# facebookresearch/FRL-Distributed-ML-Scaffold

Measured on NVIDIA H100. Metric: samples/sec (whole box) on synthetic 2-task Problem, higher is better.
Workload: dtype bf16

## Files before the change

frl-distributed-ml-scaffold_b200/_native.py:

```python
import ctypes as C
import os
import subprocess
from typing import Optional, Sequence

import torch

_HERE = os.path.dirname(os.path.abspath(__file__))
CSRC_DIR = os.path.join(_HERE, "csrc")
LIB_PATH = os.path.join(CSRC_DIR, "libfrl_b200.so")

F32, BF16, U8, I64 = 0, 1, 2, 3
LOSS_MSE, LOSS_CE = 0, 1
FP8_E4M3, FP8_E5M2 = 0, 1
FP8_DTYPE = {FP8_E4M3: torch.float8_e4m3fn, FP8_E5M2: torch.float8_e5m2}
MAX_TASKS = 8

_DTYPE_CODE = {torch.float32: F32, torch.bfloat16: BF16, torch.uint8: U8, torch.bool: U8,
               torch.int64: I64}


class NativeLibraryError(RuntimeError):
    pass


class TaskDesc(C.Structure):
    _fields_ = [
        ("kind", C.c_int32), ("out_dtype", C.c_int32), ("tgt_dtype", C.c_int32),
        ("ignore_index", C.c_int32),
        ("out", C.c_void_p), ("tgt", C.c_void_p), ("mask", C.c_void_p), ("dout", C.c_void_p),
        ("rows", C.c_int64), ("cols", C.c_int64), ("mask_inner", C.c_int64),
        ("weight", C.c_float), ("_pad", C.c_float),
    ]


class GradSeg(C.Structure):
    _fields_ = [("g", C.c_void_p), ("arena_off", C.c_int64), ("numel", C.c_int64),
                ("g_dtype", C.c_int32), ("_pad", C.c_int32)]


_vp, _i, _i64, _f, _d = C.c_void_p, C.c_int, C.c_int64, C.c_float, C.c_double
SIGNATURES = {
    "frl_abi_version": (_i, []),
    "frl_last_error": (C.c_char_p, []),
    "frl_launch_count": (C.c_uint64, []),
    "frl_launch_count_reset": (None, []),
    "frl_device_sm_count": (_i, []),
    "frl_device_arch": (_i, []),
# ... 29 lines not shown
    "frl_gather_lines": (_i, [_vp, _i64, _i64, _vp, _i64, _vp, _vp, _i64, _i64, _i, _i, _vp]),
    "frl_gather_pool_create": (_vp, [_i]),
    "frl_gather_pool_destroy": (None, [_vp]),
    "frl_gather_pool_threads": (_i, [_vp]),
    "frl_gather_pool_submit": (_i64, [_vp, _vp, _i64, _vp, _vp, _i64, _i64]),
    "frl_gather_pool_submit_f32_to_bf16": (_i64, [_vp, _vp, _i64, _vp, _vp, _i64, _i64]),
    "frl_gather_pool_wait": (_i, [_vp, _i64]),
    "frl_nvls_sgd": (_i, [_vp, _vp, _vp, _vp, _i64, _i, _i, _vp, _i, _vp, _i, _d, _d, _d, _d, _d, _vp, _i, _i, _i, _vp]),
    "frl_nvls_adam": (_i, [_vp, _vp, _vp, _vp, _vp, _vp, _i64, _i, _i, _vp, _i, _vp, _i, _d, _d, _d, _d, _d,
                           _i64, _d, _vp, _i, _i, _vp]),
    "frl_nvls_rmsprop": (_i, [_vp, _vp, _vp, _vp, _vp, _i64, _i, _i, _vp, _i, _vp, _i, _d, _d, _d, _d, _d, _d,
                              _vp, _i, _i, _vp]),
    "frl_nvls_barrier": (_i, [_vp, _i, _i, _i, _vp]),
    "frl_fp8_amax": (_i, [_vp, _i64, _i, _vp, _vp]),
    "frl_fp8_quantize": (_i, [_vp, _i64, _i64, _i, _vp, _i, _vp, _vp, _vp, _vp]),
}

_lib: Optional[C.CDLL] = None


def build(verbose: bool = False) -> str:
    cmd = ["make", "-C", CSRC_DIR, "-j8"]
    res = subprocess.run(cmd, capture_output=True, text=True)
    if verbose or res.returncode != 0:
        print(res.stdout)
        print(res.stderr)
    if res.returncode != 0:
        raise NativeLibraryError("building libfrl_b200.so failed:\n" + res.stderr[-4000:])
    return LIB_PATH

# ... 301 lines not shown
    _check(lib().frl_fp8_amax(_ptr(src), src.numel(), dtype_code(src.dtype), _ptr(amax_out), _stream()),
           "frl_fp8_amax")


def fp8_quantize(src, amax, fmt: int, dst=None, dst_t=None, inv_scale_out=None) -> None:
    rows, cols = src.shape
    want = FP8_DTYPE[fmt]
    assert src.is_contiguous() and amax.dtype == torch.float32 and inv_scale_out.dtype == torch.float32
    assert dst is None or (dst.shape == (rows, cols) and dst.dtype == want and dst.is_contiguous())
    assert dst_t is None or (dst_t.shape == (cols, rows) and dst_t.dtype == want and dst_t.is_contiguous())
    _check(lib().frl_fp8_quantize(_ptr(src), rows, cols, dtype_code(src.dtype), _ptr(amax), fmt, _ptr(dst),
                                  _ptr(dst_t), _ptr(inv_scale_out), _stream()), "frl_fp8_quantize")



def gather_rows(src_pinned, idx_dev, dst, max_blocks: int = 64) -> None:
    assert src_pinned.is_pinned() and src_pinned.is_contiguous() and dst.is_contiguous()
    row_bytes = src_pinned[0].numel() * src_pinned.element_size() if src_pinned.shape[0] else 0
    _check(lib().frl_gather_rows(_ptr(src_pinned), src_pinned.shape[0], _ptr(idx_dev), _ptr(dst),
                                 idx_dev.numel(), row_bytes, max_blocks, _stream()),
           "frl_gather_rows")


def _row_bytes(src) -> int:
    return src[0].numel() * src.element_size() if src.shape[0] else 0


def gather_rows_tma(src_pinned, idx_dev, dst, max_blocks: int = 0) -> None:
    assert src_pinned.is_pinned() and src_pinned.is_contiguous() and dst.is_contiguous()
    _check(lib().frl_gather_rows_tma(_ptr(src_pinned), src_pinned.shape[0], _ptr(idx_dev), _ptr(dst),
# ... 77 lines not shown
```

frl-distributed-ml-scaffold_b200/arena_linear.py:

```python
import os
import types
from collections import Counter
from typing import List, Optional

import torch
import torch.nn as nn
import torch.nn.functional as F

from . import _native
from .types import Precision

KERNELS = _native

FP8_MULTIPLE = 16


def fp8_site_qualifies(uses_lp: bool, in_features: int, out_features: int) -> bool:
    return bool(uses_lp) and in_features % FP8_MULTIPLE == 0 and out_features % FP8_MULTIPLE == 0


def fp8_call_qualifies(x: torch.Tensor) -> bool:
    if x.dim() == 0 or x.shape[-1] == 0 or x.dtype not in (torch.bfloat16, torch.float32):
        return False
    m = x.numel() // x.shape[-1]
    return m > 0 and m % FP8_MULTIPLE == 0 and (not x.is_contiguous() or x.data_ptr() % 16 == 0)


# ... 33 lines not shown
            KERNELS.colsum(dz2, pipe.arena.grad_view(site.bslot),
                           accumulate=not site.bstate.first_touch(pipe.step_id))
        site.backward_done(pipe)
        return dx, None, None, None, None
    dw = _fp8_mm(dztq, xtq, sdz, sx) if ctx.needs_input_grad[1] else None
    db = dz2.sum(0) if (ctx.has_bias and ctx.needs_input_grad[2]) else None
    return dx, dw, db, None, None


class _ArenaLinearFn(torch.autograd.Function):
    @staticmethod
    def forward(ctx, x, weight, bias, site):
        ctx.site = site
        ctx.has_bias = bias is not None
        ctx.save_for_backward(x, weight)
        if x.dim() <= 2:
            return F.linear(x, weight, bias)
        y = torch.empty(*x.shape[:-1], weight.shape[0], dtype=x.dtype, device=x.device)
        x2 = x.reshape(-1, x.shape[-1])
        if bias is not None:
            torch.addmm(bias, x2, weight.t(), out=y.view(-1, weight.shape[0]))
        else:
            torch.mm(x2, weight.t(), out=y.view(-1, weight.shape[0]))
        return y

    @staticmethod
    @torch.autograd.function.once_differentiable
    def backward(ctx, dy):
        x, weight = ctx.saved_tensors
        site = ctx.site
        dx = dy.matmul(weight) if ctx.needs_input_grad[0] else None
        dy2 = dy.reshape(-1, dy.shape[-1])
        x2 = x.reshape(-1, x.shape[-1])
        pipe = site.pipeline
        if pipe is not None and pipe.step_open:
            site.weight_grad(pipe, dy2, x2)
            if ctx.has_bias and site.bslot is not None:
                if not dy2.is_contiguous():
                    dy2 = dy2.contiguous()
                KERNELS.colsum(dy2, pipe.arena.grad_view(site.bslot),
                               accumulate=not site.bstate.first_touch(pipe.step_id))
            site.backward_done(pipe)
            return dx, None, None, None
        dw = dy2.t().mm(x2) if ctx.needs_input_grad[1] else None
        db = dy2.sum(0) if (ctx.has_bias and ctx.needs_input_grad[2]) else None
        return dx, dw, db, None


class _ArenaLinearReluFn(torch.autograd.Function):

    @staticmethod
    def forward(ctx, x, weight, bias, site):
        ctx.site = site
        x2 = x.reshape(-1, x.shape[-1])
        y = torch.empty(*x.shape[:-1], weight.shape[0], dtype=x.dtype, device=x.device)
        torch._addmm_activation(bias, x2, weight.t(), use_gelu=False, out=y.view(-1, weight.shape[0]))
        ctx.save_for_backward(x, weight, y)
        return y

    @staticmethod
    @torch.autograd.function.once_differentiable
    def backward(ctx, dy):
        x, weight, y = ctx.saved_tensors
        site = ctx.site
        dy2 = dy.reshape(-1, dy.shape[-1])
        if not dy2.is_contiguous():
            dy2 = dy2.contiguous()
        y2 = y.reshape(-1, y.shape[-1])
        x2 = x.reshape(-1, x.shape[-1])
        pipe = site.pipeline
        if pipe is not None and pipe.step_open and (dy2.is_cuda or KERNELS is not _native):
            dz = torch.empty_like(dy2)
            KERNELS.drelu_colsum(dy2, y2, dz, pipe.arena.grad_view(site.bslot),
                                 accumulate=not site.bstate.first_touch(pipe.step_id))
            dx = dz.matmul(weight).view_as(x) if ctx.needs_input_grad[0] else None
            site.weight_grad(pipe, dz, x2)
            site.backward_done(pipe)
            return dx, None, None, None
        dz = dy2 * (y2 > 0).to(dy2.dtype)
        dx = dz.matmul(weight).view_as(x) if ctx.needs_input_grad[0] else None
        dw = dz.t().mm(x2) if ctx.needs_input_grad[1] else None
        db = dz.sum(0) if ctx.needs_input_grad[2] else None
        return dx, dw, db, None


class _Fp8LinearFn(torch.autograd.Function):

    @staticmethod
    def forward(ctx, x, weight, bias, site, for_backward):
        ctx.site = site
        ctx.has_bias = bias is not None
        ctx.x_shape = x.shape
        xq, xtq, sx, wq, wtq, sw = _fp8_operands(x, weight, for_backward)
        y = torch.empty(*x.shape[:-1], weight.shape[0], dtype=torch.bfloat16, device=x.device)
        _fp8_mm(xq, wq, sx, sw, bias=bias, out=y.view(-1, weight.shape[0]))
        if for_backward:
# ... 37 lines not shown
        if pipe is not None and pipe.step_open:
            dz = torch.empty_like(dy2)
            KERNELS.drelu_colsum(dy2, y2, dz, pipe.arena.grad_view(site.bslot),
                                 accumulate=not site.bstate.first_touch(pipe.step_id))
            return _fp8_backward(ctx, site, dz, False)
        return _fp8_backward(ctx, site, dy2 * (y2 > 0).to(dy2.dtype), True)


class _ArenaMultiHeadFn(torch.autograd.Function):

    @staticmethod
    def forward(ctx, x, site, *params):
        ctx.site = site
        ctx.save_for_backward(x)
        ctx.n_heads = len(params) // 2
        return tuple(F.linear(x, params[2 * i], params[2 * i + 1]) for i in range(ctx.n_heads))

    @staticmethod
    @torch.autograd.function.once_differentiable
    def backward(ctx, *dys):
        (x,) = ctx.saved_tensors
        site = ctx.site
        pipe = site.pipeline
        dy = torch.cat(dys, dim=1)
        dx = dy.matmul(site.weight_cat()) if ctx.needs_input_grad[0] else None
        none = (None,) * (2 * ctx.n_heads)
        if pipe is not None and pipe.step_open:
            gw = site.grad_weight_cat()
            if site.heads[0].wstate.first_touch(pipe.step_id):
                torch.mm(dy.t(), x, out=gw)
            else:
                gw.addmm_(dy.t(), x)
            for h in site.heads[1:]:
                h.wstate.first_touch(pipe.step_id)
            gb = site.grad_bias_cat()
            if gb is not None:
                first = site.heads[0].bstate.first_touch(pipe.step_id)
                for h in site.heads[1:]:
                    h.bstate.first_touch(pipe.step_id)
                KERNELS.colsum(dy, gb, accumulate=not first)
            else:
                for h, dyi in zip(site.heads, dys):
                    KERNELS.colsum(dyi.contiguous(), pipe.arena.grad_view(h.bslot),
                                   accumulate=not h.bstate.first_touch(pipe.step_id))
            for h in site.heads:
                h.backward_done(pipe)
            return (dx, None) + none
        grads = []
        for i, dyi in enumerate(dys):
            grads += [dyi.t().mm(x) if ctx.needs_input_grad[2 + 2 * i] else None,
                      dyi.sum(0) if ctx.needs_input_grad[3 + 2 * i] else None]
        return (dx, None) + tuple(grads)


class MultiHeadSite:

    def __init__(self, model, heads: List["LinearSite"], pipeline) -> None:
        self.model = model
        self.heads = heads
        self.pipeline = pipeline
        arena = pipeline.arena
        self.rows = sum(h.module.out_features for h in heads)
        self.cols = heads[0].module.in_features
        self._w_lo = heads[0].wslot.offset
        ends = [h.wslot.end for h in heads]
        starts = [h.wslot.offset for h in heads]
        assert all(e == s for e, s in zip(ends[:-1], starts[1:])), "head weights are not adjacent"
        self._w_hi = ends[-1]
        b_adjacent = all(h.bslot.end == n.bslot.offset for h, n in zip(heads[:-1], heads[1:]))
        self._b = (heads[0].bslot.offset, heads[-1].bslot.end) if b_adjacent else None
        self._arena = arena

    def weight_cat(self) -> torch.Tensor:
        a = self._arena
        store = a.lp if self.heads[0].wslot.uses_lp else a.master
        return store[self._w_lo:self._w_hi].view(self.rows, self.cols)

    def grad_weight_cat(self) -> torch.Tensor:
        return self._arena.grad[self._w_lo:self._w_hi].view(self.rows, self.cols)

    def grad_bias_cat(self) -> Optional[torch.Tensor]:
        return None if self._b is None else self._arena.grad[self._b[0]:self._b[1]]


def head_layout_groups(model: nn.Module) -> List[List[nn.Parameter]]:
    from .model import MultiTaskModel
    if type(model) is not MultiTaskModel or os.environ.get("FRL_B200_FUSE_HEADS", "1") == "0":
        return []
    heads = list(model.additional_layers)
    if len(heads) < 2 or any(type(h) is not nn.Linear or h.bias is None for h in heads):
        return []
    if len({h.in_features for h in heads}) != 1 or len({id(h.weight) for h in heads}) != len(heads):
        return []
    return [[h.weight for h in heads], [h.bias for h in heads]]
# ... 45 lines not shown
        self.module = module
        self.wslot = wslot
        self.bslot = bslot
        self.pipeline = pipeline
        self.relu = None
        self.multihead = None
        self.fp8 = False
        states = pipeline.slot_states
        self.wstate = states.setdefault(wslot.index, SlotState())
        self.bstate = states.setdefault(bslot.index, SlotState()) if bslot is not None else None

    def weight_grad(self, pipe, dz: torch.Tensor, x2: torch.Tensor) -> None:
        gw = pipe.arena.grad_view(self.wslot)
        st = self.wstate
        if not st.first_touch(pipe.step_id):
            gw.addmm_(dz.t(), x2)
            return
        rows = pipe.row_split(self.wslot)
        if rows and st.fwd_gen == pipe.forward_gen and st.fwd_count == 1:
            torch.mm(dz[:, :rows].t(), x2, out=gw[:rows])
            pipe.rows_ready(self.wslot, rows)
            torch.mm(dz[:, rows:].t(), x2, out=gw[rows:])
        else:
            torch.mm(dz.t(), x2, out=gw)

    def weight_grad_fp8(self, pipe, dztq, xtq, s_dz, s_x) -> None:
        gw = pipe.arena.grad_view(self.wslot)
        st = self.wstate
        if not st.first_touch(pipe.step_id):
            gw.add_(_fp8_mm(dztq, xtq, s_dz, s_x))
            return
        rows = pipe.row_split(self.wslot)
        if rows and rows % FP8_MULTIPLE == 0 and st.fwd_gen == pipe.forward_gen and st.fwd_count == 1:
            _fp8_mm(dztq[:rows], xtq, s_dz, s_x, out=gw[:rows])
            pipe.rows_ready(self.wslot, rows)
            _fp8_mm(dztq[rows:], xtq, s_dz, s_x, out=gw[rows:])
        else:
            _fp8_mm(dztq, xtq, s_dz, s_x, out=gw)

# ... 144 lines not shown
```

frl-distributed-ml-scaffold_b200/criteria.py:

```python
from abc import ABC, abstractmethod
from typing import Dict, List, Optional, Sequence, Tuple

import numpy as np
import torch
import torch.nn as nn
import torch.nn.functional as F
import torch.nn.modules.loss as L

from . import _native
from .types import LossType

KERNELS = _native



class MaskedLoss(L._Loss):

    def __init__(self, loss_layer, reduction: str = "mean") -> None:
        super().__init__(reduction=reduction)
        self.loss_layer = loss_layer

    def forward(self, *inputs) -> torch.Tensor:
        output, target, mask = inputs
        assert not target.requires_grad
# ... 115 lines not shown

def _descs(plan: _Plan, outs: Sequence[torch.Tensor], douts: Optional[Sequence[torch.Tensor]]):
    descs = []
    keep = []
    for i, tp in enumerate(plan.tasks):
        out = outs[i]
        tgt = plan.targets[i].contiguous()
        mask = plan.masks[i]
        keep.append(tgt)
        d = _native.TaskDesc()
        d.kind = tp.kind
        d.out_dtype = _native.dtype_code(out.dtype)
        d.tgt_dtype = _native.dtype_code(tgt.dtype)
        d.ignore_index = tp.ignore_index
        d.out = out.data_ptr()
        d.tgt = tgt.data_ptr()
        if tp.kind == _native.LOSS_MSE:
            d.rows, d.cols = 1, max(out.numel(), 1)
            if out.dim() >= 2:
                d.rows, d.cols = out.shape[0], max(out.numel() // max(out.shape[0], 1), 1)
        else:
            d.rows, d.cols = out.shape[0], out.shape[1]
        d.mask = None
        d.mask_inner = 1
        if mask is not None:
            mask = mask.contiguous()
            keep.append(mask)
            d.mask = mask.data_ptr()
            d.mask_inner = max(out.numel() // max(mask.numel(), 1), 1)
        d.dout = douts[i].data_ptr() if douts is not None else None
        d.weight = plan.weights[i]
        descs.append(d)
    return _native.make_task_array(descs), keep


class _FusedLosses(torch.autograd.Function):

    @staticmethod
    def forward(ctx, plan: _Plan, _unused, *outputs):
        outs = [o.contiguous() for o in outputs[:plan.n]]
        dev = outs[0].device
        losses = torch.empty(1 + plan.n, dtype=torch.float32, device=dev)
        aux = torch.empty(plan.n, dtype=torch.float32, device=dev)
        n_lse = sum(o.shape[0] for o, tp in zip(outs, plan.tasks) if tp.kind == _native.LOSS_CE)
        lse = torch.empty(max(n_lse, 1), dtype=torch.float32, device=dev)
        arr, keep = _descs(plan, outs, None)
        KERNELS.criteria_forward(arr, plan.n, losses, aux, lse, plan.sink, plan.nan_flag,
                                 _scratch_for(dev, plan.n))
        ctx.plan = plan
        ctx.save_for_backward(aux, lse, *outs)
        ctx.set_materialize_grads(True)
        return losses

    @staticmethod
    @torch.autograd.function.once_differentiable
    def backward(ctx, grad_losses):
        plan = ctx.plan
        aux, lse, *outs = ctx.saved_tensors
        gl = grad_losses.contiguous().float()
        douts = [torch.empty_like(o) for o in outs]
        arr, keep = _descs(plan, outs, douts)
        KERNELS.criteria_backward(arr, plan.n, gl, aux, lse)
        return (None, None, *douts)


_path_logged = set()


def _log_path_once(modules, fused: bool) -> None:
    key = (tuple(type(m).__name__ for m in modules), fused)
    if key not in _path_logged:
        _path_logged.add(key)
        import logging
        logging.getLogger(__name__).info(
            "criterion path for loss modules %s: %s", list(key[0]),
            "fused kernels (frl_criteria_forward / _backward, one launch each)" if fused else
            "composed torch ops — outside the fused kernels' domain (MSE / CrossEntropy with mean "
            "reduction, optionally inside MaskedLoss)")
# ... 176 lines not shown
```

frl-distributed-ml-scaffold_b200/csrc/criteria.cu:

```cuda
#include "frl_common.cuh"

namespace frl {

constexpr int kCThreads = 256;
constexpr int kCWarps = kCThreads / 32;
constexpr int kCMaxBlocksPerTask = 528;
constexpr int kCVecPerLane = 8;
constexpr int kCRowChunk = 32 * 4 * kCVecPerLane;

struct CritParams {
    frl_task_desc t[FRL_MAX_TASKS];
    int nblk[FRL_MAX_TASKS];
    int blk_start[FRL_MAX_TASKS];
    int part_off[FRL_MAX_TASKS];
    int64_t lse_off[FRL_MAX_TASKS];
    int n_tasks;
    int total_blocks;
};

struct CritScratchHeader {
    unsigned int ticket;
    unsigned int _pad[3];
};
static inline int64_t crit_scratch_bytes(int T) {
// ... 40 lines not shown
template <> struct Raw4<float> { f32x4 v; };
template <> struct Raw4<__nv_bfloat16> { bf16x4 v; };
__device__ __forceinline__ Raw4<float> ldraw4(const float* base, int64_t e) {
    return Raw4<float>{*reinterpret_cast<const f32x4*>(base + e)};
}
__device__ __forceinline__ Raw4<__nv_bfloat16> ldraw4(const __nv_bfloat16* base, int64_t e) {
    return Raw4<__nv_bfloat16>{*reinterpret_cast<const bf16x4*>(base + e)};
}
__device__ __forceinline__ f32x4 cvt4(const Raw4<float>& r) { return r.v; }
__device__ __forceinline__ f32x4 cvt4(const Raw4<__nv_bfloat16>& r) {
    return f32x4{bf16lo(r.v.a), bf16hi(r.v.a), bf16lo(r.v.b), bf16hi(r.v.b)};
}
__device__ __forceinline__ void fill_neg_inf(Raw4<float>& r) { r.v = f32x4{-INFINITY, -INFINITY, -INFINITY, -INFINITY}; }
__device__ __forceinline__ void fill_neg_inf(Raw4<__nv_bfloat16>& r) { r.v = bf16x4{0xff80ff80u, 0xff80ff80u}; }

__device__ __forceinline__ bool vec_ok(const frl_task_desc& t) {
    const int esz = t.out_dtype == FRL_F32 ? 4 : 2;
    return (t.cols % 4 == 0) && ((reinterpret_cast<uintptr_t>(t.out) % (4 * esz)) == 0) &&
           (t.dout == nullptr || (reinterpret_cast<uintptr_t>(t.dout) % (4 * esz)) == 0);
}

template <typename OT>
__device__ __forceinline__ void mse_partial(const frl_task_desc& t, int blk, int nblk,
                                            float& sum, float& nsel) {
    const int64_t n = t.rows * t.cols;
    const int64_t stride = static_cast<int64_t>(nblk) * kCThreads;
    float s = 0.f, c = 0.f;
    for (int64_t e = static_cast<int64_t>(blk) * kCThreads + threadIdx.x; e < n; e += stride) {
        if (t.mask && t.mask[e / t.mask_inner] == 0) continue;
        const float d = ldf<OT>(t.out, e) - ld_any(t.tgt, t.tgt_dtype, e);
        s = fmaf(d, d, s);
        c += 1.f;
    }
    sum = s;
    nsel = c;
}

template <typename OT>
__device__ __forceinline__ void ce_partial(const frl_task_desc& t, int blk, int nblk, float* lse_out,
                                           float& sum, float& nsel, float& nvalid) {
    const int lane = threadIdx.x & 31, warp = threadIdx.x >> 5;
    const int64_t C = t.cols;
    const bool vec = vec_ok(t);
    const int64_t* labels = static_cast<const int64_t*>(t.tgt);
    float s_loss = 0.f, s_sel = 0.f, s_valid = 0.f;
    for (int64_t row = static_cast<int64_t>(blk) * kCWarps + warp; row < t.rows;
         row += static_cast<int64_t>(nblk) * kCWarps) {
        const int64_t r0 = row * C;
        float m = -INFINITY, se = 0.f;
        bool has_nan = false;
        if (vec && C <= kCRowChunk) {
            Raw4<OT> q[kCVecPerLane];
            const OT* base = static_cast<const OT*>(t.out);
#pragma unroll
            for (int j = 0; j < kCVecPerLane; ++j) {
                const int64_t c = lane * 4 + j * 128;
                if (c < C) q[j] = ldraw4(base, r0 + c); else fill_neg_inf(q[j]);
            }
#pragma unroll
            for (int j = 0; j < kCVecPerLane; ++j) {
                const f32x4 v = cvt4(q[j]);
                m = fmaxf(fmaxf(m, fmaxf(v.x, v.y)), fmaxf(v.z, v.w));
            }
// ... 150 lines not shown
    if (threadIdx.x == 0) {
        losses[0] = total;
        if (sink) sink[0] = total;
        if (nan_flag && (total != total)) *nan_flag = 1;
        hdr->ticket = 0;
    }
}

template <typename OT>
__device__ __forceinline__ void mse_bwd(const frl_task_desc& t, int blk, int nblk, float coef) {
    const int64_t n = t.rows * t.cols;
    const int64_t stride = static_cast<int64_t>(nblk) * kCThreads;
    for (int64_t e = static_cast<int64_t>(blk) * kCThreads + threadIdx.x; e < n; e += stride) {
        float d = 0.f;
        if (!(t.mask && t.mask[e / t.mask_inner] == 0))
            d = (ldf<OT>(t.out, e) - ld_any(t.tgt, t.tgt_dtype, e)) * coef;
        stf<OT>(t.dout, e, d);
    }
}

template <typename OT>
__device__ __forceinline__ void ce_bwd(const frl_task_desc& t, int blk, int nblk, const float* lse,
                                       float coef) {
    const int lane = threadIdx.x & 31, warp = threadIdx.x >> 5;
    const int64_t C = t.cols;
    const bool vec = vec_ok(t);
    const int64_t* labels = static_cast<const int64_t*>(t.tgt);
    for (int64_t row = static_cast<int64_t>(blk) * kCWarps + warp; row < t.rows;
         row += static_cast<int64_t>(nblk) * kCWarps) {
        const int64_t r0 = row * C;
        const int64_t y = labels[row];
        const bool use = ((t.mask == nullptr) || (t.mask[row] != 0)) &&
                         (y != static_cast<int64_t>(t.ignore_index));
        const float k = use ? coef : 0.f;
        const float l = lse[row];
        if (vec) {
            for (int64_t cb = 0; cb < C; cb += kCRowChunk) {
                f32x4 v[kCVecPerLane];
#pragma unroll
                for (int j = 0; j < kCVecPerLane; ++j) {
                    const int64_t c = cb + lane * 4 + j * 128;
                    if (c < C) v[j] = ld4<OT>(t.out, r0 + c);
                }
#pragma unroll
                for (int j = 0; j < kCVecPerLane; ++j) {
// ... 39 lines not shown
}

static int build_params(const frl_task_desc* tasks, int T, bool backward, CritParams& P, int& max_blk,
                        const char* name) {
    FRL_REQUIRE(tasks != nullptr && T >= 1, FRL_E_ARG, "%s: no tasks", name);
    FRL_REQUIRE(T <= FRL_MAX_TASKS, FRL_E_TOO_MANY, "%s: at most %d tasks", name, FRL_MAX_TASKS);
    int off = 0;
    int64_t lse_off = 0;
    max_blk = 1;
    P.n_tasks = T;
    for (int i = 0; i < T; ++i) {
        const frl_task_desc& t = tasks[i];
        FRL_REQUIRE(t.kind == FRL_LOSS_MSE || t.kind == FRL_LOSS_CE, FRL_E_ARG, "%s: task %d kind", name, i);
        FRL_REQUIRE(t.out_dtype == FRL_F32 || t.out_dtype == FRL_BF16, FRL_E_DTYPE, "%s: task %d out dtype", name, i);
        FRL_REQUIRE(t.rows >= 0 && t.cols >= 1, FRL_E_ARG, "%s: task %d shape", name, i);
        FRL_REQUIRE(t.rows == 0 || (t.out && t.tgt), FRL_E_ARG, "%s: task %d null out/tgt", name, i);
        FRL_REQUIRE(!backward || t.rows == 0 || t.dout, FRL_E_ARG, "%s: task %d null dout", name, i);
        if (t.kind == FRL_LOSS_MSE) {
            FRL_REQUIRE(t.tgt_dtype == FRL_F32 || t.tgt_dtype == FRL_BF16, FRL_E_DTYPE, "%s: task %d tgt dtype", name, i);
            FRL_REQUIRE(!t.mask || t.mask_inner >= 1, FRL_E_ARG, "%s: task %d mask_inner", name, i);
        } else {
            FRL_REQUIRE(t.tgt_dtype == FRL_I64, FRL_E_DTYPE, "%s: task %d CE labels must be int64", name, i);
            FRL_REQUIRE(!t.mask || t.mask_inner == t.cols, FRL_E_ARG, "%s: task %d CE mask is per row", name, i);
        }
        P.t[i] = t;
        int64_t work_blocks;
        if (t.kind == FRL_LOSS_MSE) work_blocks = (t.rows * t.cols + kCThreads * 8 - 1) / (kCThreads * 8);
        else                        work_blocks = (t.rows + kCWarps - 1) / kCWarps;
        if (work_blocks < 1) work_blocks = 1;
        if (work_blocks > kCMaxBlocksPerTask) work_blocks = kCMaxBlocksPerTask;
// ... 55 lines not shown
```

include/frl_b200.h:

```cpp
#ifndef FRL_B200_H
#define FRL_B200_H

#include <stdint.h>

#ifdef __cplusplus
extern "C" {
#endif

#define FRL_ABI_VERSION 1

enum { FRL_F32 = 0, FRL_BF16 = 1, FRL_U8 = 2, FRL_I64 = 3 };
enum { FRL_E_ARG = -1, FRL_E_ALIGN = -2, FRL_E_DTYPE = -3, FRL_E_TOO_MANY = -4 };

int          frl_abi_version(void);
const char*  frl_last_error(void);
uint64_t     frl_launch_count(void);
void         frl_launch_count_reset(void);
int          frl_device_sm_count(void);
int          frl_device_arch(void);


int frl_sgd_momentum(float* p, const void* g, float* buf, void* p_lp, int64_t n,
                     double lr, double mu, double dampening, double wd,
                     double grad_scale, const float* grad_scale_dev, const float* dyn,
// ... 65 lines not shown
enum { FRL_LOSS_MSE = 0, FRL_LOSS_CE = 1 };

typedef struct frl_task_desc {
    int32_t     kind;
    int32_t     out_dtype;
    int32_t     tgt_dtype;
    int32_t     ignore_index;
    const void* out;
    const void* tgt;
    const uint8_t* mask;
    void*       dout;
    int64_t     rows;
    int64_t     cols;
    int64_t     mask_inner;
    float       weight;
    float       _pad;
} frl_task_desc;

int64_t frl_criteria_scratch_bytes(int n_tasks);

int frl_criteria_forward(const frl_task_desc* tasks_host, int n_tasks,
                         float* losses, float* aux, float* lse,
                         float* sink_mapped, int32_t* nan_flag_mapped,
                         void* scratch, void* stream);

int frl_criteria_backward(const frl_task_desc* tasks_host, int n_tasks,
                          const float* grad_losses, const float* aux, const float* lse,
                          void* stream);

int frl_preproc_affine(const void* src, int src_dtype, void* dst, int dst_dtype, int64_t n,
                       int64_t inner, int64_t channels, const float* scale, const float* bias,
                       void* stream);

enum { FRL_AUG_RRC = 0, FRL_AUG_PAD_CROP = 1, FRL_AUG_CENTER_RESIZE = 2, FRL_AUG_CENTER_CROP = 3 };
int frl_augment_images(const void* src, int64_t batch, int channels, int height, int width,
                       const int64_t* idx, uint64_t seed, int epoch, int mode,
                       double smin, double smax, double rmin, double rmax, double eval_crop, int pad,
                       int flip, const float* scale, const float* bias, void* dst, int dst_dtype,
                       int out_h, int out_w, int32_t* params_out, void* stream);

int frl_cast_scale(const void* src, int src_dtype, void* dst, int dst_dtype, int64_t n,
                   float scale, void* stream);

// ... 56 lines not shown
```

Before: 1.922 million.

## Route linear GEMMs through cached cuBLASLt plans with fused bias/ReLU epilogues

Adds a native cuBLASLt GEMM wrapper with a per-shape algorithm cache and routes every bf16 linear forward and backward matmul through it, using bias and bias+ReLU epilogues. Multi-head forward now writes all heads into one concatenated output with a single GEMM, and the criteria kernels accept strided column-block outputs, avoiding a contiguous copy and a torch.cat. The goal is fewer launches and copies, at the cost of per-call Python descriptor construction and descriptor/layout creation on every cuBLASLt call, which adds host overhead.

Measured after the change: 1.937 million (median of 6 runs). About the same (+0.7%).

```diff
diff --git a/frl-distributed-ml-scaffold_b200/_native.py b/frl-distributed-ml-scaffold_b200/_native.py
--- a/frl-distributed-ml-scaffold_b200/_native.py
+++ b/frl-distributed-ml-scaffold_b200/_native.py
@@ -29,8 +29,15 @@
         ("ignore_index", C.c_int32),
         ("out", C.c_void_p), ("tgt", C.c_void_p), ("mask", C.c_void_p), ("dout", C.c_void_p),
         ("rows", C.c_int64), ("cols", C.c_int64), ("mask_inner", C.c_int64),
-        ("weight", C.c_float), ("_pad", C.c_float),
+        ("weight", C.c_float), ("out_ld", C.c_int32),
     ]
+
+
+class GemmDesc(C.Structure):
+    _fields_ = [("a", C.c_void_p), ("b", C.c_void_p), ("d", C.c_void_p), ("bias", C.c_void_p),
+                ("m", C.c_int64), ("n", C.c_int64), ("k", C.c_int64),
+                ("lda", C.c_int64), ("ldb", C.c_int64), ("ldd", C.c_int64),
+                ("trans_a", C.c_int32), ("trans_b", C.c_int32), ("epilogue", C.c_int32), ("beta", C.c_int32)]
 
 
 class GradSeg(C.Structure):
@@ -90,6 +97,8 @@
     "frl_nvls_barrier": (_i, [_vp, _i, _i, _i, _vp]),
     "frl_fp8_amax": (_i, [_vp, _i64, _i, _vp, _vp]),
     "frl_fp8_quantize": (_i, [_vp, _i64, _i64, _i, _vp, _i, _vp, _vp, _vp, _vp]),
+    "frl_gemm_plan": (_i, [C.POINTER(GemmDesc), _vp, _i64, _vp, _i, _vp, _vp, _vp]),
+    "frl_gemm_run": (_i, [C.POINTER(GemmDesc), _vp, _vp, _i64, _vp]),
 }
 
 _lib: Optional[C.CDLL] = None
@@ -421,6 +430,122 @@
 
 
 
+GEMM_EPI_NONE, GEMM_EPI_BIAS, GEMM_EPI_BIAS_RELU = 0, 1, 2
+GEMM_ALGO_BYTES = 64
+GEMM_WORKSPACE_BYTES = 32 << 20
+
+
+def _align(ptr: int) -> int:
+    a = 256
+    while a > 2 and ptr % a:
+        a >>= 1
+    return a
+
+
+def _gemm_operand(t: torch.Tensor):
+    r, c = t.shape
+    s0, s1 = t.stride()
+    if s1 == 1 and s0 >= max(c, 1):
+        return 0, s0, t
+    if s0 == 1 and s1 >= max(r, 1):
+        return 1, s1, t
+    return 0, max(c, 1), t.contiguous()
+
+
+class GemmPlanner:
+
+    def __init__(self) -> None:
+        self.plans = {}
+        self._workspace = {}
+
+    @staticmethod
+    def key(desc: GemmDesc, device) -> tuple:
+        return (device, desc.m, desc.n, desc.k, desc.trans_a, desc.trans_b, desc.lda, desc.ldb, desc.ldd,
+                desc.epilogue, desc.beta, _align(desc.a), _align(desc.b), _align(desc.d))
+
+    def stream(self) -> int:
+        return _stream()
+
+    def workspace(self, device, stream: int) -> torch.Tensor:
+        ws = self._workspace.get((device, stream))
+        if ws is None:
+            ws = self._workspace[(device, stream)] = torch.empty(GEMM_WORKSPACE_BYTES, dtype=torch.uint8,
+                                                                 device=device)
+        return ws
+
+    def select(self, desc: GemmDesc, device, stream: int, ws: torch.Tensor, timed: bool):
+        algo = C.create_string_buffer(GEMM_ALGO_BYTES)
+        info = (C.c_int32 * 2)()
+        scratch, sptr = None, None
+        if timed:
+            nbytes = ((desc.m - 1) * desc.ldd + desc.n) * 2
+            scratch = torch.zeros(nbytes + 256, dtype=torch.uint8, device=device)
+            base = scratch.data_ptr()
+            sptr = base + ((desc.d - base) % 256)
+        _check(lib().frl_gemm_plan(C.byref(desc), ws.data_ptr(), ws.numel(), sptr, int(timed), algo, info, stream),
+               "frl_gemm_plan")
+        del scratch
+        return algo.raw, int(info[0]), int(info[1])
+
+    def run(self, desc: GemmDesc, device) -> None:
+        stream = self.stream()
+        ws = self.workspace(device, stream)
+        key = self.key(desc, device)
+        plan = self.plans.get(key)
+        if plan is None:
+            plan = self.plans[key] = self.select(desc, device, stream, ws, timed=False)
+        self.launch(desc, plan[0], ws, stream)
+
+    def launch(self, desc: GemmDesc, algo: bytes, ws: torch.Tensor, stream: int) -> None:
+        _check(lib().frl_gemm_run(C.byref(desc), algo, ws.data_ptr(), ws.numel(), stream), "frl_gemm_run")
+
+
+PLANNER = GemmPlanner()
+
+
+def gemm_desc(a, b, out, bias=None, relu=False, accumulate=False):
+    if not (a.dtype == b.dtype == out.dtype == torch.bfloat16) or (bias is not None and bias.dtype != torch.bfloat16):
+        raise NativeLibraryError("gemm: operands, output and bias must be bf16")
+    if a.dim() != 2 or b.dim() != 2 or out.dim() != 2:
+        raise NativeLibraryError("gemm: 2-D operands expected")
+    m, k = a.shape
+    n = b.shape[1]
+    if b.shape[0] != k or tuple(out.shape) != (m, n):
+        raise NativeLibraryError(f"gemm: shapes {tuple(a.shape)} @ {tuple(b.shape)} -> {tuple(out.shape)}")
+    if out.stride(1) != 1 or out.stride(0) < n:
+        raise NativeLibraryError("gemm: output rows must be dense")
+    if (relu and bias is None) or (accumulate and (bias is not None or relu)):
+        raise NativeLibraryError("gemm: ReLU needs a bias, accumulation takes neither")
+    if bias is not None and (bias.dim() != 1 or bias.numel() != n or not bias.is_contiguous()):
+        raise NativeLibraryError("gemm: bias must be a contiguous [n] vector")
+    ta, lda, a = _gemm_operand(a)
+    tb, ldb, b = _gemm_operand(b)
+    d = GemmDesc()
+    d.a, d.b, d.d, d.bias = a.data_ptr(), b.data_ptr(), out.data_ptr(), _ptr(bias)
+    d.m, d.n, d.k, d.lda, d.ldb, d.ldd = m, n, k, lda, ldb, out.stride(0)
+    d.trans_a, d.trans_b = ta, tb
+    d.epilogue = GEMM_EPI_NONE if bias is None else (GEMM_EPI_BIAS_RELU if relu else GEMM_EPI_BIAS)
+    d.beta = int(bool(accumulate))
+    return d, (a, b)
+
+
+def gemm(a, b, out, *, bias=None, relu=False, accumulate=False) -> None:
+    if out.numel() == 0:
+        return
+    if a.shape[1] == 0:
+        if not accumulate:
+            out.zero_()
+        if bias is not None:
+            out.add_(bias)
+        if relu:
+            out.relu_()
+        return
+    desc, keep = gemm_desc(a, b, out, bias, relu, accumulate)
+    PLANNER.run(desc, out.device)
+    del keep
+
+
+
 def gather_rows(src_pinned, idx_dev, dst, max_blocks: int = 64) -> None:
     assert src_pinned.is_pinned() and src_pinned.is_contiguous() and dst.is_contiguous()
     row_bytes = src_pinned[0].numel() * src_pinned.element_size() if src_pinned.shape[0] else 0
diff --git a/frl-distributed-ml-scaffold_b200/arena_linear.py b/frl-distributed-ml-scaffold_b200/arena_linear.py
--- a/frl-distributed-ml-scaffold_b200/arena_linear.py
+++ b/frl-distributed-ml-scaffold_b200/arena_linear.py
@@ -1,16 +1,39 @@
 import os
 import types
+import itertools
 from collections import Counter
 from typing import List, Optional
 
 import torch
 import torch.nn as nn
-import torch.nn.functional as F
 
 from . import _native
 from .types import Precision
 
 KERNELS = _native
+
+
+def _mm(a, b, out, bias=None, relu=False, accumulate=False):
+    if out.is_cuda and out.dtype == torch.bfloat16:
+        _native.gemm(a, b, out, bias=bias, relu=relu, accumulate=accumulate)
+    elif accumulate:
+        out.addmm_(a, b)
+    elif relu:
+        torch._addmm_activation(bias, a, b, use_gelu=False, out=out)
+    elif bias is not None:
+        torch.addmm(bias, a, b, out=out)
+    else:
+        torch.mm(a, b, out=out)
+    return out
+
+
+def _rows_2d(t: torch.Tensor) -> torch.Tensor:
+    return t.view(-1, t.shape[-1])
+
+
+def _new_out(shape, like: torch.Tensor) -> torch.Tensor:
+    return torch.empty(tuple(shape), dtype=like.dtype, device=like.device)
+
 
 FP8_MULTIPLE = 16
 
@@ -74,14 +97,8 @@
         ctx.site = site
         ctx.has_bias = bias is not None
         ctx.save_for_backward(x, weight)
-        if x.dim() <= 2:
-            return F.linear(x, weight, bias)
         y = torch.empty(*x.shape[:-1], weight.shape[0], dtype=x.dtype, device=x.device)
-        x2 = x.reshape(-1, x.shape[-1])
-        if bias is not None:
-            torch.addmm(bias, x2, weight.t(), out=y.view(-1, weight.shape[0]))
-        else:
-            torch.mm(x2, weight.t(), out=y.view(-1, weight.shape[0]))
+        _mm(x.reshape(-1, x.shape[-1]), weight.t(), _rows_2d(y), bias=bias)
         return y
 
     @staticmethod
@@ -89,9 +106,12 @@
     def backward(ctx, dy):
         x, weight = ctx.saved_tensors
         site = ctx.site
-        dx = dy.matmul(weight) if ctx.needs_input_grad[0] else None
         dy2 = dy.reshape(-1, dy.shape[-1])
         x2 = x.reshape(-1, x.shape[-1])
+        dx = None
+        if ctx.needs_input_grad[0]:
+            dx = torch.empty(x.shape, dtype=dy.dtype, device=dy.device)
+            _mm(dy2, weight, _rows_2d(dx))
         pipe = site.pipeline
         if pipe is not None and pipe.step_open:
             site.weight_grad(pipe, dy2, x2)
@@ -102,7 +122,7 @@
                                accumulate=not site.bstate.first_touch(pipe.step_id))
             site.backward_done(pipe)
             return dx, None, None, None
-        dw = dy2.t().mm(x2) if ctx.needs_input_grad[1] else None
+        dw = _mm(dy2.t(), x2, _new_out(weight.shape, dy2)) if ctx.needs_input_grad[1] else None
         db = dy2.sum(0) if (ctx.has_bias and ctx.needs_input_grad[2]) else None
         return dx, dw, db, None
 
@@ -114,7 +134,7 @@
         ctx.site = site
         x2 = x.reshape(-1, x.shape[-1])
         y = torch.empty(*x.shape[:-1], weight.shape[0], dtype=x.dtype, device=x.device)
-        torch._addmm_activation(bias, x2, weight.t(), use_gelu=False, out=y.view(-1, weight.shape[0]))
+        _mm(x2, weight.t(), _rows_2d(y), bias=bias, relu=True)
         ctx.save_for_backward(x, weight, y)
         return y
 
@@ -133,13 +153,13 @@
             dz = torch.empty_like(dy2)
             KERNELS.drelu_colsum(dy2, y2, dz, pipe.arena.grad_view(site.bslot),
                                  accumulate=not site.bstate.first_touch(pipe.step_id))
-            dx = dz.matmul(weight).view_as(x) if ctx.needs_input_grad[0] else None
+            dx = _mm(dz, weight, _new_out(x2.shape, dz)).view_as(x) if ctx.needs_input_grad[0] else None
             site.weight_grad(pipe, dz, x2)
             site.backward_done(pipe)
             return dx, None, None, None
         dz = dy2 * (y2 > 0).to(dy2.dtype)
-        dx = dz.matmul(weight).view_as(x) if ctx.needs_input_grad[0] else None
-        dw = dz.t().mm(x2) if ctx.needs_input_grad[1] else None
+        dx = _mm(dz, weight, _new_out(x2.shape, dz)).view_as(x) if ctx.needs_input_grad[0] else None
+        dw = _mm(dz.t(), x2, _new_out(weight.shape, dz)) if ctx.needs_input_grad[1] else None
         db = dz.sum(0) if ctx.needs_input_grad[2] else None
         return dx, dw, db, None
 
@@ -207,7 +227,14 @@
         ctx.site = site
         ctx.save_for_backward(x)
         ctx.n_heads = len(params) // 2
-        return tuple(F.linear(x, params[2 * i], params[2 * i + 1]) for i in range(ctx.n_heads))
+        y = torch.empty(x.shape[0], site.rows, dtype=x.dtype, device=x.device)
+        gb = site.bias_cat()
+        if gb is not None:
+            _mm(x, site.weight_cat().t(), y, bias=gb)
+        else:
+            for i, (lo, hi) in enumerate(site.col_ranges):
+                _mm(x, params[2 * i].t(), y[:, lo:hi], bias=params[2 * i + 1])
+        return tuple(y[:, lo:hi] for lo, hi in site.col_ranges)
 
     @staticmethod
     @torch.autograd.function.once_differentiable
@@ -215,15 +242,14 @@
         (x,) = ctx.saved_tensors
         site = ctx.site
         pipe = site.pipeline
-        dy = torch.cat(dys, dim=1)
-        dx = dy.matmul(site.weight_cat()) if ctx.needs_input_grad[0] else None
+        dy = column_blocks(dys)
+        if dy is None:
+            dy = torch.cat(dys, dim=1)
+        dx = _mm(dy, site.weight_cat(), _new_out(x.shape, dy)) if ctx.needs_input_grad[0] else None
         none = (None,) * (2 * ctx.n_heads)
         if pipe is not None and pipe.step_open:
-            gw = site.grad_weight_cat()
-            if site.heads[0].wstate.first_touch(pipe.step_id):
-                torch.mm(dy.t(), x, out=gw)
-            else:
-                gw.addmm_(dy.t(), x)
+            first = site.heads[0].wstate.first_touch(pipe.step_id)
+            _mm(dy.t(), x, site.grad_weight_cat(), accumulate=not first)
             for h in site.heads[1:]:
                 h.wstate.first_touch(pipe.step_id)
             gb = site.grad_bias_cat()
@@ -241,9 +267,24 @@
             return (dx, None) + none
         grads = []
         for i, dyi in enumerate(dys):
-            grads += [dyi.t().mm(x) if ctx.needs_input_grad[2 + 2 * i] else None,
+            grads += [_mm(dyi.t(), x, _new_out((dyi.shape[1], x.shape[1]), dyi))
+                      if ctx.needs_input_grad[2 + 2 * i] else None,
                       dyi.sum(0) if ctx.needs_input_grad[3 + 2 * i] else None]
         return (dx, None) + tuple(grads)
+
+
+def column_blocks(dys) -> Optional[torch.Tensor]:
+    if any(d.dim() != 2 for d in dys):
+        return None
+    d0 = dys[0]
+    width = sum(d.shape[1] for d in dys)
+    col = 0
+    for d in dys:
+        if (d.dtype != d0.dtype or d.device != d0.device or d.shape[0] != d0.shape[0]
+                or d.stride() != (width, 1) or d.data_ptr() != d0.data_ptr() + col * d.element_size()):
+            return None
+        col += d.shape[1]
+    return d0.as_strided((d0.shape[0], width), (width, 1))
 
 
 class MultiHeadSite:
@@ -254,6 +295,8 @@
         self.pipeline = pipeline
         arena = pipeline.arena
         self.rows = sum(h.module.out_features for h in heads)
+        ends = list(itertools.accumulate(h.module.out_features for h in heads))
+        self.col_ranges = list(zip([0] + ends[:-1], ends))
         self.cols = heads[0].module.in_features
         self._w_lo = heads[0].wslot.offset
         ends = [h.wslot.end for h in heads]
@@ -271,6 +314,13 @@
 
     def grad_weight_cat(self) -> torch.Tensor:
         return self._arena.grad[self._w_lo:self._w_hi].view(self.rows, self.cols)
+
+    def bias_cat(self) -> Optional[torch.Tensor]:
+        if self._b is None:
+            return None
+        a = self._arena
+        store = a.lp if self.heads[0].bslot.uses_lp else a.master
+        return store[self._b[0]:self._b[1]]
 
     def grad_bias_cat(self) -> Optional[torch.Tensor]:
         return None if self._b is None else self._arena.grad[self._b[0]:self._b[1]]
@@ -346,15 +396,15 @@
         gw = pipe.arena.grad_view(self.wslot)
         st = self.wstate
         if not st.first_touch(pipe.step_id):
-            gw.addmm_(dz.t(), x2)
+            _mm(dz.t(), x2, gw, accumulate=True)
             return
         rows = pipe.row_split(self.wslot)
         if rows and st.fwd_gen == pipe.forward_gen and st.fwd_count == 1:
-            torch.mm(dz[:, :rows].t(), x2, out=gw[:rows])
+            _mm(dz[:, :rows].t(), x2, gw[:rows])
             pipe.rows_ready(self.wslot, rows)
-            torch.mm(dz[:, rows:].t(), x2, out=gw[rows:])
+            _mm(dz[:, rows:].t(), x2, gw[rows:])
         else:
-            torch.mm(dz.t(), x2, out=gw)
+            _mm(dz.t(), x2, gw)
 
     def weight_grad_fp8(self, pipe, dztq, xtq, s_dz, s_x) -> None:
         gw = pipe.arena.grad_view(self.wslot)
diff --git a/frl-distributed-ml-scaffold_b200/criteria.py b/frl-distributed-ml-scaffold_b200/criteria.py
--- a/frl-distributed-ml-scaffold_b200/criteria.py
+++ b/frl-distributed-ml-scaffold_b200/criteria.py
@@ -8,6 +8,7 @@
 import torch.nn.modules.loss as L
 
 from . import _native
+from .arena_linear import column_blocks
 from .types import LossType
 
 KERNELS = _native
@@ -153,6 +154,7 @@
         d.tgt_dtype = _native.dtype_code(tgt.dtype)
         d.ignore_index = tp.ignore_index
         d.out = out.data_ptr()
+        d.out_ld = 0 if out.is_contiguous() else out.stride(0)
         d.tgt = tgt.data_ptr()
         if tp.kind == _native.LOSS_MSE:
             d.rows, d.cols = 1, max(out.numel(), 1)
@@ -177,7 +179,9 @@
 
     @staticmethod
     def forward(ctx, plan: _Plan, _unused, *outputs):
-        outs = [o.contiguous() for o in outputs[:plan.n]]
+        outs = list(outputs[:plan.n])
+        if column_blocks(outs) is None or outs[0].stride(0) >= 2 ** 31:
+            outs = [o.contiguous() for o in outs]
         dev = outs[0].device
         losses = torch.empty(1 + plan.n, dtype=torch.float32, device=dev)
         aux = torch.empty(plan.n, dtype=torch.float32, device=dev)
@@ -197,10 +201,21 @@
         plan = ctx.plan
         aux, lse, *outs = ctx.saved_tensors
         gl = grad_losses.contiguous().float()
-        douts = [torch.empty_like(o) for o in outs]
+        douts = _grad_outputs(outs)
         arr, keep = _descs(plan, outs, douts)
         KERNELS.criteria_backward(arr, plan.n, gl, aux, lse)
         return (None, None, *douts)
+
+
+def _grad_outputs(outs: List[torch.Tensor]) -> List[torch.Tensor]:
+    base = column_blocks(outs)
+    if base is None:
+        return [torch.empty_like(o) for o in outs]
+    g = torch.empty(base.shape, dtype=base.dtype, device=base.device)
+    cols = [0]
+    for o in outs:
+        cols.append(cols[-1] + o.shape[1])
+    return [g[:, lo:hi] for lo, hi in zip(cols[:-1], cols[1:])]
 
 
 _path_logged = set()
diff --git a/frl-distributed-ml-scaffold_b200/csrc/criteria.cu b/frl-distributed-ml-scaffold_b200/csrc/criteria.cu
--- a/frl-distributed-ml-scaffold_b200/csrc/criteria.cu
+++ b/frl-distributed-ml-scaffold_b200/csrc/criteria.cu
@@ -78,9 +78,16 @@
 __device__ __forceinline__ void fill_neg_inf(Raw4<float>& r) { r.v = f32x4{-INFINITY, -INFINITY, -INFINITY, -INFINITY}; }
 __device__ __forceinline__ void fill_neg_inf(Raw4<__nv_bfloat16>& r) { r.v = bf16x4{0xff80ff80u, 0xff80ff80u}; }
 
+__device__ __forceinline__ int64_t row_ld(const frl_task_desc& t) { return t.out_ld > 0 ? t.out_ld : t.cols; }
+__device__ __forceinline__ int64_t out_off(const frl_task_desc& t, int64_t e) {
+    if (t.out_ld <= 0 || t.out_ld == t.cols) return e;
+    const int64_t r = e / t.cols;
+    return r * t.out_ld + (e - r * t.cols);
+}
+
 __device__ __forceinline__ bool vec_ok(const frl_task_desc& t) {
     const int esz = t.out_dtype == FRL_F32 ? 4 : 2;
-    return (t.cols % 4 == 0) && ((reinterpret_cast<uintptr_t>(t.out) % (4 * esz)) == 0) &&
+    return (t.cols % 4 == 0) && (row_ld(t) % 4 == 0) && ((reinterpret_cast<uintptr_t>(t.out) % (4 * esz)) == 0) &&
            (t.dout == nullptr || (reinterpret_cast<uintptr_t>(t.dout) % (4 * esz)) == 0);
 }
 
@@ -92,7 +99,7 @@
     float s = 0.f, c = 0.f;
     for (int64_t e = static_cast<int64_t>(blk) * kCThreads + threadIdx.x; e < n; e += stride) {
         if (t.mask && t.mask[e / t.mask_inner] == 0) continue;
-        const float d = ldf<OT>(t.out, e) - ld_any(t.tgt, t.tgt_dtype, e);
+        const float d = ldf<OT>(t.out, out_off(t, e)) - ld_any(t.tgt, t.tgt_dtype, e);
         s = fmaf(d, d, s);
         c += 1.f;
     }
@@ -110,7 +117,7 @@
     float s_loss = 0.f, s_sel = 0.f, s_valid = 0.f;
     for (int64_t row = static_cast<int64_t>(blk) * kCWarps + warp; row < t.rows;
          row += static_cast<int64_t>(nblk) * kCWarps) {
-        const int64_t r0 = row * C;
+        const int64_t r0 = row * row_ld(t);
         float m = -INFINITY, se = 0.f;
         bool has_nan = false;
         if (vec && C <= kCRowChunk) {
@@ -291,8 +298,8 @@
     for (int64_t e = static_cast<int64_t>(blk) * kCThreads + threadIdx.x; e < n; e += stride) {
         float d = 0.f;
         if (!(t.mask && t.mask[e / t.mask_inner] == 0))
-            d = (ldf<OT>(t.out, e) - ld_any(t.tgt, t.tgt_dtype, e)) * coef;
-        stf<OT>(t.dout, e, d);
+            d = (ldf<OT>(t.out, out_off(t, e)) - ld_any(t.tgt, t.tgt_dtype, e)) * coef;
+        stf<OT>(t.dout, out_off(t, e), d);
     }
 }
 
@@ -305,7 +312,7 @@
     const int64_t* labels = static_cast<const int64_t*>(t.tgt);
     for (int64_t row = static_cast<int64_t>(blk) * kCWarps + warp; row < t.rows;
          row += static_cast<int64_t>(nblk) * kCWarps) {
-        const int64_t r0 = row * C;
+        const int64_t r0 = row * row_ld(t);
         const int64_t y = labels[row];
         const bool use = ((t.mask == nullptr) || (t.mask[row] != 0)) &&
                          (y != static_cast<int64_t>(t.ignore_index));
@@ -375,6 +382,7 @@
         FRL_REQUIRE(t.kind == FRL_LOSS_MSE || t.kind == FRL_LOSS_CE, FRL_E_ARG, "%s: task %d kind", name, i);
         FRL_REQUIRE(t.out_dtype == FRL_F32 || t.out_dtype == FRL_BF16, FRL_E_DTYPE, "%s: task %d out dtype", name, i);
         FRL_REQUIRE(t.rows >= 0 && t.cols >= 1, FRL_E_ARG, "%s: task %d shape", name, i);
+        FRL_REQUIRE(t.out_ld == 0 || t.out_ld >= t.cols, FRL_E_ARG, "%s: task %d out_ld < cols", name, i);
         FRL_REQUIRE(t.rows == 0 || (t.out && t.tgt), FRL_E_ARG, "%s: task %d null out/tgt", name, i);
         FRL_REQUIRE(!backward || t.rows == 0 || t.dout, FRL_E_ARG, "%s: task %d null dout", name, i);
         if (t.kind == FRL_LOSS_MSE) {
diff --git a/frl-distributed-ml-scaffold_b200/csrc/gemm.cu b/frl-distributed-ml-scaffold_b200/csrc/gemm.cu
--- /dev/null
+++ b/frl-distributed-ml-scaffold_b200/csrc/gemm.cu
@@ -0,0 +1,179 @@
+#include <cublasLt.h>
+#include <mutex>
+#include <string.h>
+
+#include "frl_common.cuh"
+
+namespace frl {
+
+static_assert(sizeof(cublasLtMatmulAlgo_t) <= FRL_GEMM_ALGO_BYTES, "frl_gemm_algo too small");
+
+constexpr int kGemmMaxCandidates = 8;
+constexpr int kGemmTimedReps = 5;
+
+static cublasLtHandle_t lt_handle() {
+    static std::mutex mu;
+    static cublasLtHandle_t h = nullptr;
+    std::lock_guard<std::mutex> lock(mu);
+    if (h == nullptr && cublasLtCreate(&h) != CUBLAS_STATUS_SUCCESS) h = nullptr;
+    return h;
+}
+
+static int align_bytes(const void* p) {
+    const uintptr_t a = reinterpret_cast<uintptr_t>(p);
+    int al = 256;
+    while (al > 2 && (a % al) != 0) al >>= 1;
+    return al;
+}
+
+struct LtCall {
+    cublasLtMatmulDesc_t op = nullptr;
+    cublasLtMatrixLayout_t la = nullptr, lb = nullptr, ld = nullptr;
+    ~LtCall() {
+        if (ld) cublasLtMatrixLayoutDestroy(ld);
+        if (lb) cublasLtMatrixLayoutDestroy(lb);
+        if (la) cublasLtMatrixLayoutDestroy(la);
+        if (op) cublasLtMatmulDescDestroy(op);
+    }
+};
+
+#define FRL_LT(call, what)                                                                   \
+    do {                                                                                     \
+        const cublasStatus_t s_ = (call);                                                    \
+        FRL_REQUIRE(s_ == CUBLAS_STATUS_SUCCESS, FRL_E_ARG, "%s: %s failed (cublasStatus %d)", \
+                    name, what, static_cast<int>(s_));                                       \
+    } while (0)
+
+static int check_desc(const frl_gemm_desc* g, const char* name) {
+    FRL_REQUIRE(g != nullptr, FRL_E_ARG, "%s: null descriptor", name);
+    FRL_REQUIRE(g->m >= 1 && g->n >= 1 && g->k >= 1, FRL_E_ARG, "%s: empty problem %lld x %lld x %lld", name,
+                (long long)g->m, (long long)g->n, (long long)g->k);
+    FRL_REQUIRE(g->a && g->b && g->d, FRL_E_ARG, "%s: null operand", name);
+    FRL_REQUIRE(g->lda >= (g->trans_a ? g->m : g->k) && g->ldb >= (g->trans_b ? g->k : g->n) && g->ldd >= g->n,
+                FRL_E_ARG, "%s: leading dimension too small", name);
+    FRL_REQUIRE(g->epilogue == FRL_GEMM_EPI_NONE || g->epilogue == FRL_GEMM_EPI_BIAS ||
+                g->epilogue == FRL_GEMM_EPI_BIAS_RELU, FRL_E_ARG, "%s: epilogue %d", name, g->epilogue);
+    FRL_REQUIRE(g->epilogue == FRL_GEMM_EPI_NONE || g->bias, FRL_E_ARG, "%s: bias epilogue without bias", name);
+    FRL_REQUIRE(g->beta == 0 || (g->beta == 1 && g->epilogue == FRL_GEMM_EPI_NONE), FRL_E_ARG,
+                "%s: beta must be 0, or 1 without an epilogue", name);
+    return 0;
+}
+
+static int make_call(const frl_gemm_desc* g, LtCall& c, const char* name) {
+    const cublasOperation_t ta = g->trans_b ? CUBLAS_OP_T : CUBLAS_OP_N;
+    const cublasOperation_t tb = g->trans_a ? CUBLAS_OP_T : CUBLAS_OP_N;
+    FRL_LT(cublasLtMatmulDescCreate(&c.op, CUBLAS_COMPUTE_32F, CUDA_R_32F), "MatmulDescCreate");
+    FRL_LT(cublasLtMatmulDescSetAttribute(c.op, CUBLASLT_MATMUL_DESC_TRANSA, &ta, sizeof(ta)), "TRANSA");
+    FRL_LT(cublasLtMatmulDescSetAttribute(c.op, CUBLASLT_MATMUL_DESC_TRANSB, &tb, sizeof(tb)), "TRANSB");
+    if (g->epilogue != FRL_GEMM_EPI_NONE) {
+        const cublasLtEpilogue_t epi = g->epilogue == FRL_GEMM_EPI_BIAS ? CUBLASLT_EPILOGUE_BIAS
+                                                                        : CUBLASLT_EPILOGUE_RELU_BIAS;
+        FRL_LT(cublasLtMatmulDescSetAttribute(c.op, CUBLASLT_MATMUL_DESC_EPILOGUE, &epi, sizeof(epi)), "EPILOGUE");
+        FRL_LT(cublasLtMatmulDescSetAttribute(c.op, CUBLASLT_MATMUL_DESC_BIAS_POINTER, &g->bias, sizeof(g->bias)),
+               "BIAS_POINTER");
+    }
+    FRL_LT(cublasLtMatrixLayoutCreate(&c.la, CUDA_R_16BF, g->trans_b ? g->k : g->n, g->trans_b ? g->n : g->k, g->ldb),
+           "layout A");
+    FRL_LT(cublasLtMatrixLayoutCreate(&c.lb, CUDA_R_16BF, g->trans_a ? g->m : g->k, g->trans_a ? g->k : g->m, g->lda),
+           "layout B");
+    FRL_LT(cublasLtMatrixLayoutCreate(&c.ld, CUDA_R_16BF, g->n, g->m, g->ldd), "layout D");
+    return 0;
+}
+
+static int launch(const frl_gemm_desc* g, const LtCall& c, const cublasLtMatmulAlgo_t* algo, void* d,
+                  void* workspace, int64_t ws_bytes, cudaStream_t s, const char* name) {
+    const float alpha = 1.f, beta = static_cast<float>(g->beta);
+    FRL_LT(cublasLtMatmul(lt_handle(), c.op, &alpha, g->b, c.la, g->a, c.lb, &beta, d, c.ld, d, c.ld, algo,
+                          workspace, static_cast<size_t>(ws_bytes), s),
+           "cublasLtMatmul");
+    return 0;
+}
+
+}
+
+using namespace frl;
+
+extern "C" int frl_gemm_plan(const frl_gemm_desc* g, void* workspace, int64_t workspace_bytes, void* scratch_d,
+                             int timed, void* algo_out, int32_t* info_out, void* stream) {
+    const char* name = "frl_gemm_plan";
+    if (const int rc = check_desc(g, name)) return rc;
+    FRL_REQUIRE(algo_out && info_out, FRL_E_ARG, "%s: null outputs", name);
+    FRL_REQUIRE(workspace_bytes >= 0 && (workspace || workspace_bytes == 0), FRL_E_ARG, "%s: workspace", name);
+    cublasLtHandle_t h = lt_handle();
+    FRL_REQUIRE(h != nullptr, FRL_E_ARG, "%s: cublasLtCreate failed", name);
+    LtCall c;
+    if (const int rc = make_call(g, c, name)) return rc;
+
+    cublasLtMatmulPreference_t pref = nullptr;
+    FRL_LT(cublasLtMatmulPreferenceCreate(&pref), "PreferenceCreate");
+    struct PrefGuard { cublasLtMatmulPreference_t p; ~PrefGuard() { cublasLtMatmulPreferenceDestroy(p); } } pg{pref};
+    const uint64_t ws = static_cast<uint64_t>(workspace_bytes);
+    FRL_LT(cublasLtMatmulPreferenceSetAttribute(pref, CUBLASLT_MATMUL_PREF_MAX_WORKSPACE_BYTES, &ws, sizeof(ws)),
+           "MAX_WORKSPACE_BYTES");
+    const uint32_t schemes = CUBLASLT_REDUCTION_SCHEME_COMPUTE_TYPE;
+    FRL_LT(cublasLtMatmulPreferenceSetAttribute(pref, CUBLASLT_MATMUL_PREF_REDUCTION_SCHEME_MASK, &schemes,
+                                                sizeof(schemes)), "REDUCTION_SCHEME_MASK");
+    const uint32_t al_a = align_bytes(g->b), al_b = align_bytes(g->a), al_d = align_bytes(g->d);
+    FRL_LT(cublasLtMatmulPreferenceSetAttribute(pref, CUBLASLT_MATMUL_PREF_MIN_ALIGNMENT_A_BYTES, &al_a, sizeof(al_a)), "ALIGN_A");
+    FRL_LT(cublasLtMatmulPreferenceSetAttribute(pref, CUBLASLT_MATMUL_PREF_MIN_ALIGNMENT_B_BYTES, &al_b, sizeof(al_b)), "ALIGN_B");
+    FRL_LT(cublasLtMatmulPreferenceSetAttribute(pref, CUBLASLT_MATMUL_PREF_MIN_ALIGNMENT_C_BYTES, &al_d, sizeof(al_d)), "ALIGN_C");
+    FRL_LT(cublasLtMatmulPreferenceSetAttribute(pref, CUBLASLT_MATMUL_PREF_MIN_ALIGNMENT_D_BYTES, &al_d, sizeof(al_d)), "ALIGN_D");
+
+    cublasLtMatmulHeuristicResult_t res[kGemmMaxCandidates];
+    int n_res = 0;
+    FRL_LT(cublasLtMatmulAlgoGetHeuristic(h, c.op, c.la, c.lb, c.ld, c.ld, pref, kGemmMaxCandidates, res, &n_res),
+           "AlgoGetHeuristic");
+    FRL_REQUIRE(n_res >= 1, FRL_E_ARG, "%s: cuBLASLt offers no algorithm for %lld x %lld x %lld", name,
+                (long long)g->m, (long long)g->n, (long long)g->k);
+
+    const cudaStream_t s = static_cast<cudaStream_t>(stream);
+    cudaStreamCaptureStatus cap = cudaStreamCaptureStatusNone;
+    if (cudaStreamIsCapturing(s, &cap) != cudaSuccess) cap = cudaStreamCaptureStatusActive;
+    int best = 0;
+    float best_ms = -1.f;
+    if (timed && scratch_d && n_res > 1 && cap == cudaStreamCaptureStatusNone) {
+        cudaEvent_t e0 = nullptr, e1 = nullptr;
+        FRL_REQUIRE(cudaEventCreate(&e0) == cudaSuccess && cudaEventCreate(&e1) == cudaSuccess, FRL_E_ARG,
+                    "%s: cudaEventCreate failed", name);
+        int rc = 0;
+        for (int i = 0; i < n_res && rc == 0; ++i) {
+            if (res[i].state != CUBLAS_STATUS_SUCCESS || res[i].workspaceSize > ws) continue;
+            rc = launch(g, c, &res[i].algo, scratch_d, workspace, workspace_bytes, s, name);
+            cudaEventRecord(e0, s);
+            for (int r = 0; r < kGemmTimedReps && rc == 0; ++r)
+                rc = launch(g, c, &res[i].algo, scratch_d, workspace, workspace_bytes, s, name);
+            cudaEventRecord(e1, s);
+            float ms = 0.f;
+            if (rc == 0 && cudaEventSynchronize(e1) == cudaSuccess && cudaEventElapsedTime(&ms, e0, e1) == cudaSuccess &&
+                (best_ms < 0.f || ms < best_ms)) {
+                best_ms = ms;
+                best = i;
+            }
+        }
+        cudaEventDestroy(e0);
+        cudaEventDestroy(e1);
+        if (rc) return rc;
+        const cudaError_t e = cudaGetLastError();
+        FRL_REQUIRE(e == cudaSuccess, static_cast<int>(e), "%s: timing failed: %s", name, cudaGetErrorString(e));
+    }
+    FRL_REQUIRE(res[best].workspaceSize <= ws, FRL_E_ARG, "%s: algorithm needs %zu workspace bytes", name,
+                res[best].workspaceSize);
+    memset(algo_out, 0, FRL_GEMM_ALGO_BYTES);
+    memcpy(algo_out, &res[best].algo, sizeof(cublasLtMatmulAlgo_t));
+    info_out[0] = n_res;
+    info_out[1] = best;
+    return 0;
+}
+
+extern "C" int frl_gemm_run(const frl_gemm_desc* g, const void* algo, void* workspace, int64_t workspace_bytes,
+                            void* stream) {
+    const char* name = "frl_gemm_run";
+    if (const int rc = check_desc(g, name)) return rc;
+    FRL_REQUIRE(algo != nullptr, FRL_E_ARG, "%s: null algorithm", name);
+    FRL_REQUIRE(lt_handle() != nullptr, FRL_E_ARG, "%s: cublasLtCreate failed", name);
+    LtCall c;
+    if (const int rc = make_call(g, c, name)) return rc;
+    cublasLtMatmulAlgo_t a;
+    memcpy(&a, algo, sizeof(a));
+    return launch(g, c, &a, g->d, workspace, workspace_bytes, static_cast<cudaStream_t>(stream), name);
+}
diff --git a/include/frl_b200.h b/include/frl_b200.h
--- a/include/frl_b200.h
+++ b/include/frl_b200.h
@@ -103,7 +103,7 @@
     int64_t     cols;
     int64_t     mask_inner;
     float       weight;
-    float       _pad;
+    int32_t     out_ld;
 } frl_task_desc;
 
 int64_t frl_criteria_scratch_bytes(int n_tasks);
@@ -116,6 +116,26 @@
 int frl_criteria_backward(const frl_task_desc* tasks_host, int n_tasks,
                           const float* grad_losses, const float* aux, const float* lse,
                           void* stream);
+
+#define FRL_GEMM_ALGO_BYTES 64
+enum { FRL_GEMM_EPI_NONE = 0, FRL_GEMM_EPI_BIAS = 1, FRL_GEMM_EPI_BIAS_RELU = 2 };
+
+typedef struct frl_gemm_desc {
+    const void* a;
+    const void* b;
+    void*       d;
+    const void* bias;
+    int64_t     m, n, k;
+    int64_t     lda, ldb, ldd;
+    int32_t     trans_a, trans_b;
+    int32_t     epilogue;
+    int32_t     beta;
+} frl_gemm_desc;
+
+int frl_gemm_plan(const frl_gemm_desc* g, void* workspace, int64_t workspace_bytes, void* scratch_d,
+                  int timed, void* algo_out, int32_t* info_out, void* stream);
+int frl_gemm_run(const frl_gemm_desc* g, const void* algo, void* workspace, int64_t workspace_bytes,
+                 void* stream);
 
 int frl_preproc_affine(const void* src, int src_dtype, void* dst, int dst_dtype, int64_t n,
                        int64_t inner, int64_t channels, const float* scale, const float* bias,
```
